# sfu-rsl/FastTrack

Measured on AMD Instinct MI355X. Metric: frames/sec extract+match, higher is better.
Workload: dtype u8

## Files before the change

fasttrack_amd/csrc/kernels_extract.hip:

```cpp
#include "ft_internal.h"
#include "libm_f32.h"
#include "wave_ops.h"

namespace {


struct FtMomentTab {
    unsigned W[17 * 8], M[17 * 8];
};
constexpr FtMomentTab ft_make_moment_tab() {
    constexpr int umax[16] = {15, 15, 15, 15, 14, 14, 14, 13, 13, 12, 11, 10, 9, 8, 6, 3};
    FtMomentTab t{};
    for (int av = 0; av < 16; av++)
        for (int j = 0; j < 8; j++)
            for (int k = 0; k < 4; k++) {
                const int u = -15 + 4 * j + k;
                const int au = u < 0 ? -u : u;
                if (u <= 15 && au <= umax[av]) {
                    t.W[av * 8 + j] |= (unsigned)(u + 16) << (8 * k);
                    t.M[av * 8 + j] |= 1u << (8 * k);
                }
            }
    return t;
}
// ... 140 lines not shown
                pk |= (unsigned)((r0[0] + r0[1] + r1[0] + r1[1] + 2) >> 2) << (8 * k);
            }
            gstore<unsigned>(outLevel + (unsigned)vmad24(dy, D.pitch, bx), pk);
        }
        return;
    }
    int cx0[4], cx1[4];
#pragma unroll
    for (int k = 0; k < 4; k++) {
        cx0[k] = xt[k].s - sxa;
        cx1[k] = min(xt[k].s + 1, sw - 1) - sxa;
    }
#pragma unroll
    for (int j = 0; j < 4; j++) {
        const int dy = by + j;
        if (dy > dy1) break;
        const int sy0 = min(max((int)yt[j].s, 0), sh - 1) - sya, sy1 = min(max((int)yt[j].s + 1, 0), sh - 1) - sya;
        const uint8_t *r0 = T + __mul24(sy0, ldsPitch), *r1 = T + __mul24(sy1, ldsPitch);
        unsigned pk = 0;
#pragma unroll
        for (int k = 0; k < 4; k++) {
            const int h0 = r0[cx0[k]] * xt[k].a0 + r0[cx1[k]] * xt[k].a1;
            const int h1 = r1[cx0[k]] * xt[k].a0 + r1[cx1[k]] * xt[k].a1;
            pk |= (unsigned)(((vmul24((int)yt[j].a0, h0 >> 4) >> 16) + (vmul24((int)yt[j].a1, h1 >> 4) >> 16) + 2) >> 2) << (8 * k);
        }
        gstore<unsigned>(outLevel + (unsigned)vmad24(dy, D.pitch, bx), pk);
    }
}

#define PR_COLS 128
#ifndef PR_RB
#define PR_RB 32
#endif
#ifndef PR_PF
#define PR_PF 4
#endif
typedef unsigned short ft_us2 __attribute__((ext_vector_type(2)));
typedef unsigned ft_u2 __attribute__((ext_vector_type(2)));
__device__ __forceinline__ unsigned udot2_u16(unsigned a, unsigned b) {
    return __builtin_amdgcn_udot2(__builtin_bit_cast(ft_us2, a), __builtin_bit_cast(ft_us2, b), 0u, false);
}
__device__ __forceinline__ unsigned umulhi_su(unsigned bShifted16, unsigned a) {
    unsigned r;
    asm("v_mul_hi_u32 %0, %1, %2" : "=v"(r) : "s"(bShifted16), "v"(a));
    return r;
}
template <bool AREA, bool BAND>
__device__ __forceinline__ void pyr_rows_strip(const FtGeom &g, int level, int slot, int tx, int j0, int rowEnd, int lane,
                                               const uint8_t *S, int spitch, uint8_t *pyr, const FtTap *taps, int readableEnd) {
    const FtLevelGeom &D = g.lv[level];
    const int sw = g.lv[level - 1].w, sh = g.lv[level - 1].h;
    const int dx = tx * PR_COLS + 2 * lane;
    const int nrows = min(PR_RB, (BAND ? rowEnd : D.h) - j0);
    unsigned rowW0 = 0, rowW1 = 0;
    if constexpr (!AREA) {
        const ft_u2 t = gload<ft_u2>(taps + D.ytab + j0 + min(lane, nrows - 1));
        const int sy = (int)(short)(t.x & 0xffffu);
        rowW0 = (unsigned)min(max(sy, 0), sh - 1) | ((unsigned)min(max(sy + 1, 0), sh - 1) << 16);
        rowW1 = (t.x >> 16) | (t.y << 16);
        if (lane >= nrows) rowW0 = 0xffffffffu;
    }
    const int dxa = min(dx, D.w - 1), dxb = min(dx + 1, D.w - 1);
    int sxa, sxb, cxa, cxb;
    unsigned wa, wb;
    if constexpr (AREA) {
        sxa = 2 * dxa; sxb = 2 * dxb; cxa = sxa + 1; cxb = sxb + 1;
        wa = wb = 0x00010001u;
    } else {
        const ft_u2 ta = gload<ft_u2>(taps + D.xtab + dxa), tb = gload<ft_u2>(taps + D.xtab + dxb);
        sxa = (int)(short)(ta.x & 0xffffu); sxb = (int)(short)(tb.x & 0xffffu);
        cxa = min(sxa + 1, sw - 1); cxb = min(sxb + 1, sw - 1);
        wa = (ta.x >> 16) | (ta.y << 16);
        wb = (tb.x >> 16) | (tb.y << 16);
    }
    const int base = min(sxa & ~3, readableEnd - 8);
    const unsigned selA = (unsigned)(sxa - base) | 0x0c00u | ((unsigned)(cxa - base) << 16) | 0x0c000000u;
    const unsigned selB = (unsigned)(sxb - base) | 0x0c00u | ((unsigned)(cxb - base) << 16) | 0x0c000000u;
    auto rowTap = [&](int r, int &sy0, int &sy1, unsigned &b0, unsigned &b1) {
        if constexpr (AREA) {
            sy0 = 2 * (j0 + r); sy1 = r < nrows ? sy0 + 1 : -1; b0 = b1 = 0;
        } else {
            const unsigned w0 = (unsigned)__builtin_amdgcn_readlane((int)rowW0, r), w1 = (unsigned)__builtin_amdgcn_readlane((int)rowW1, r);
            sy0 = (int)(w0 & 0xffffu); sy1 = (int)(w0 >> 16);
            b0 = w1 << 16; b1 = w1 & 0xffff0000u;
        }
    };
    int jr = 0, sy0, sy1;
    unsigned b0, b1;
    rowTap(0, sy0, sy1, b0, b1);
    int lastSy0, rLast;
    unsigned bx0, bx1;
    rowTap(nrows - 1, lastSy0, rLast, bx0, bx1);
    int r = sy0;
    const uint8_t *srcBase = S;
    uint8_t *dstBase = pyr + (size_t)slot * g.pyrPerSlot + D.off + (size_t)j0 * D.pitch;
    unsigned dOff = 0;
    const unsigned laneSrc = (unsigned)base, laneDst = (unsigned)dx;
    const bool store2 = dx + 1 < D.w, store1 = dx < D.w;
    auto run = [&](auto edgeTag) {
        constexpr bool EDGE = decltype(edgeTag)::value;
        int pfIdx = r;
        auto prefetch = [&]() -> ft_u2 {
            unsigned offS = laneSrc + (unsigned)min(pfIdx, rLast) * (unsigned)spitch;
            asm volatile("" : "+v"(offS));
            const ft_u2 v = gload<ft_u2>(srcBase + offS);
            pfIdx++;
            return v;
        };
        ft_u2 q[PR_PF];
#pragma unroll
        for (int k = 0; k < PR_PF; k++) q[k] = prefetch();
        unsigned hpA = 0, hpB = 0, hcA = 0, hcB = 0;
        auto take = [&](ft_u2 &q) {
            hpA = hcA; hpB = hcB;
            hcA = udot2_u16(__builtin_amdgcn_perm(q.y, q.x, selA), wa);
            hcB = udot2_u16(__builtin_amdgcn_perm(q.y, q.x, selB), wb);
            if constexpr (!AREA) { hcA >>= 4; hcB >>= 4; }
            q = prefetch();
        };
        auto step = [&]() {
            while (sy1 == r) {
                if (__builtin_expect(sy0 == r, 0)) {
                    hpA = hcA; hpB = hcB;
                    asm volatile("" : "+v"(hpA), "+v"(hpB));
                }
                unsigned oA, oB;
                if constexpr (AREA) {
                    oA = (hpA + hcA + 2u) >> 2; oB = (hpB + hcB + 2u) >> 2;
                } else {
                    oA = (umulhi_su(b0, hpA) + umulhi_su(b1, hcA) + 2u) >> 2;
                    oB = (umulhi_su(b0, hpB) + umulhi_su(b1, hcB) + 2u) >> 2;
                }
                unsigned offD = laneDst + dOff;
                asm volatile("" : "+v"(offD));
                if constexpr (!EDGE) {
                    gstore<unsigned short>(dstBase + offD, (unsigned short)(oA | (oB << 8)));
                } else {
                    if (store2) gstore<unsigned short>(dstBase + offD, (unsigned short)(oA | (oB << 8)));
                    else if (store1) gstore<uint8_t>(dstBase + offD, (uint8_t)oA);
                }
                dOff += (unsigned)D.pitch;
                jr++;
                rowTap(jr, sy0, sy1, b0, b1);
            }
            r++;
        };
        for (int left = rLast - r + 1; left > 0; left -= PR_PF) {
#pragma unroll
            for (int k = 0; k < PR_PF; k++) {
                take(q[k]);
                step();
            }
        }
    };
    if (tx * PR_COLS + PR_COLS <= D.w) run(std::false_type{});
    else run(std::true_type{});
}

template <bool AREA>
__global__ __launch_bounds__(64) void k_pyr_rows(FtGeom g, int level, const uint8_t *const *l0, int l0pitch, uint8_t *pyr,
                                                 const FtTap *taps, FtSlotGrid sg, int stripsX, unsigned sxMagic,
                                                 int readableEnd) {
    const int lane = threadIdx.x;
    int slot, tile;
    if (!ft_slot_block(sg, slot, tile)) return;
    const int ty = div_by(tile, sxMagic), tx = tile - ty * stripsX;
    int spitch;
    const uint8_t *S = level_ptr(g, level - 1, slot, l0, l0pitch, pyr, spitch);
    pyr_rows_strip<AREA, false>(g, level, slot, tx, ty * PR_RB, 0, lane, S, spitch, pyr, taps, readableEnd);
}

__global__ __launch_bounds__(64 * PC_WAVES) void k_pyr_cascade(FtGeom g, const uint8_t *const *l0, int l0pitch, uint8_t *pyr,
                                                              const FtTap *taps, FtSlotGrid sg, FtPyrBands pb,
                                                              int l0ReadableEnd) {
    const int lane = threadIdx.x & 63, wave = wave_index();
    int slot, band;
    if (!ft_slot_block(sg, slot, band)) return;
    const uint8_t *const frame = l0[slot];
    for (int level = 1; level < g.nlevels; level++) {
        const unsigned rr = pb.rows[level][band];
        const int r0 = (int)(rr & 0xffffu), r1 = (int)(rr >> 16);
        const int stripsX = (g.lv[level].w + PR_COLS - 1) / PR_COLS;
        const unsigned sxMagic = div_magic_small((unsigned)stripsX);
        const int n = stripsX * ((r1 - r0 + PR_RB - 1) / PR_RB);
        const int readableEnd = level == 1 ? l0ReadableEnd : g.lv[level - 1].pitch;
        const int spitch = level == 1 ? l0pitch : g.lv[level - 1].pitch;
        const uint8_t *S = level == 1 ? frame : pyr + (size_t)slot * g.pyrPerSlot + g.lv[level - 1].off;
        for (int s = wave; s < n; s += PC_WAVES) {
            const int ty = div_by(s, sxMagic), tx = s - ty * stripsX;
            const int j0 = r0 + ty * PR_RB;
            if (g.lv[level].area2x) pyr_rows_strip<true, true>(g, level, slot, tx, j0, r1, lane, S, spitch, pyr, taps, readableEnd);
            else pyr_rows_strip<false, true>(g, level, slot, tx, j0, r1, lane, S, spitch, pyr, taps, readableEnd);
        }
        if (level + 1 < g.nlevels) {
            __builtin_amdgcn_fence(__ATOMIC_RELEASE, "workgroup");
            __syncthreads();
            __builtin_amdgcn_fence(__ATOMIC_ACQUIRE, "workgroup");
        }
    }
}

typedef unsigned short fs_us2 __attribute__((ext_vector_type(2)));
__device__ __forceinline__ unsigned pk_max_u16(unsigned a, unsigned b) {
    return __builtin_bit_cast(unsigned, __builtin_elementwise_max(__builtin_bit_cast(fs_us2, a), __builtin_bit_cast(fs_us2, b)));
}
__device__ __forceinline__ unsigned pk_min_u16(unsigned a, unsigned b) {
    return __builtin_bit_cast(unsigned, __builtin_elementwise_min(__builtin_bit_cast(fs_us2, a), __builtin_bit_cast(fs_us2, b)));
}
__device__ __forceinline__ bool has_arc9(unsigned m) {
    unsigned d = m | (m << 16);
    unsigned a = d & (d >> 1);
    a &= a >> 2;
    a &= a >> 4;
    a &= d >> 8;
    return (a & 0xffffu) != 0;
}

#define FT_RING(F)                                                                                            \
    F(0, 0, 3) F(1, 1, 3) F(2, 2, 2) F(3, 3, 1) F(4, 3, 0) F(5, 3, -1) F(6, 2, -2) F(7, 1, -3) F(8, 0, -3)    \
    F(9, -1, -3) F(10, -2, -2) F(11, -3, -1) F(12, -3, 0) F(13, -3, 1) F(14, -2, 2) F(15, -1, 3)

__device__ __forceinline__ int fast_score(int v, const int p[16]) {
    int mn3[16], mx3[16];
#pragma unroll
    for (int k = 0; k < 16; k++) {
        mn3[k] = min(min(p[k], p[(k + 1) & 15]), p[(k + 2) & 15]);
        mx3[k] = max(max(p[k], p[(k + 1) & 15]), p[(k + 2) & 15]);
    }
    int mn9[16], mx9[16];
#pragma unroll
    for (int k = 0; k < 16; k++) {
        mn9[k] = min(min(mn3[k], mn3[(k + 3) & 15]), mn3[(k + 6) & 15]);
        mx9[k] = max(max(mx3[k], mx3[(k + 3) & 15]), mx3[(k + 6) & 15]);
    }
    int darkest = max(max(mn9[0], mn9[1]), mn9[2]), brightest = min(min(mx9[0], mx9[1]), mx9[2]);
#pragma unroll
    for (int k = 3; k < 15; k += 2) {
        darkest = max(max(darkest, mn9[k]), mn9[k + 1]);
        brightest = min(min(brightest, mx9[k]), mx9[k + 1]);
    }
    darkest = max(darkest, mn9[15]);
    brightest = min(brightest, mx9[15]);
    return max(v - brightest, darkest - v) - 1;
}

__device__ __forceinline__ unsigned pk_min3_h(unsigned a, unsigned b, unsigned c) {
    unsigned r;
    asm("v_pk_minimum3_f16 %0, %1, %2, %3" : "=v"(r) : "v"(a), "v"(b), "v"(c));
    return r;
}
__device__ __forceinline__ unsigned pk_max3_h(unsigned a, unsigned b, unsigned c) {
    unsigned r;
    asm("v_pk_maximum3_f16 %0, %1, %2, %3" : "=v"(r) : "v"(a), "v"(b), "v"(c));
    return r;
}
typedef short fs_s2 __attribute__((ext_vector_type(2)));
__device__ __forceinline__ unsigned fast_score2(unsigned v, const unsigned p[16]) {
    unsigned mn3[16], mx3[16];
#pragma unroll
    for (int k = 0; k < 16; k++) {
        mn3[k] = pk_min3_h(p[k], p[(k + 1) & 15], p[(k + 2) & 15]);
        mx3[k] = pk_max3_h(p[k], p[(k + 1) & 15], p[(k + 2) & 15]);
    }
    unsigned mn9[16], mx9[16];
#pragma unroll
    for (int k = 0; k < 16; k++) {
        mn9[k] = pk_min3_h(mn3[k], mn3[(k + 3) & 15], mn3[(k + 6) & 15]);
        mx9[k] = pk_max3_h(mx3[k], mx3[(k + 3) & 15], mx3[(k + 6) & 15]);
    }
    unsigned darkest = pk_max3_h(mn9[0], mn9[1], mn9[2]), brightest = pk_min3_h(mx9[0], mx9[1], mx9[2]);
#pragma unroll
    for (int k = 3; k < 15; k += 2) {
        darkest = pk_max3_h(darkest, mn9[k], mn9[k + 1]);
        brightest = pk_min3_h(brightest, mx9[k], mx9[k + 1]);
    }
    const fs_s2 dk = __builtin_bit_cast(fs_s2, pk_max3_h(darkest, mn9[15], mn9[15]));
    const fs_s2 br = __builtin_bit_cast(fs_s2, pk_min3_h(brightest, mx9[15], mx9[15]));
    const fs_s2 vv = __builtin_bit_cast(fs_s2, v);
    const fs_s2 sc = __builtin_elementwise_max(vv - br, dk - vv) - (fs_s2)(1);
    return __builtin_bit_cast(unsigned, sc);
}

#ifndef FC_CAND
#define FC_CAND 512
#endif
#ifndef FC_XCD_RUN
#define FC_XCD_RUN 8
#endif
#ifndef FC_UNROLL
#define FC_UNROLL 2
#endif
#ifndef FC_ROWS
#define FC_ROWS 4
#endif
#ifndef FC_NMS_REG
#define FC_NMS_REG 2
#endif
#ifndef FC_CORN
#define FC_CORN 384
#endif
#ifndef FC_WAVES_PER_EU
#define FC_WAVES_PER_EU 1
#endif
__host__ __device__ __forceinline__ int fc_pitch(int wCell, int TP) { return TP ? TP : ((wCell + 12) & ~3); }
__host__ __device__ __forceinline__ int fc_tile_bytes(int wCell, int hCell, int TP) {
    const int t = (hCell + 6) * fc_pitch(wCell, TP), f = wCell * hCell;
    return ((t > f ? t : f) + 15) & ~15;
}
__host__ __device__ __forceinline__ int fc_score_bytes(int wCell, int hCell, int TP) { return (((hCell + 2) * fc_pitch(wCell, TP)) + 15) & ~15; }
__host__ __device__ __forceinline__ int fc_list_bytes() { return 2 * (FC_CAND + FC_CORN) + 16; }

template <int TP, bool ORDERED>
__global__ __launch_bounds__(64, FC_WAVES_PER_EU) void k_fast_cells(FtGeom g, const uint8_t *const *l0, int l0pitch, const uint8_t *pyr,
                                                   int iniTh, int minTh, int alignedLoads, int *cellCount,
                                                   uint32_t *stage, const FtCellRec *cellTab, FtSlotGrid sg, int dbg, int tileBytes,
                                                   int scoreBytesMax, FtCellRanges cr) {
    extern __shared__ __attribute__((aligned(16))) uint8_t smem[];
    const int lane = threadIdx.x;
    int slot = blockIdx.y, cellSg = 0;
    if (sg.xcdMap && !ft_slot_block(sg, slot, cellSg)) return;
    const uint8_t *img0 = l0[slot];
    const int j = (int)(blockIdx.x >> 3), xcd = (int)(blockIdx.x & 7);
    const int cj = sg.xcdMap ? cellSg : ((j / FC_XCD_RUN) * 8 + xcd) * FC_XCD_RUN + (j % FC_XCD_RUN);
    if (cj >= cr.n0 + cr.n1) return;
    const int cell = cj < cr.n0 ? cr.lo0 + cj : cr.lo1 + (cj - cr.n0);
    const FtCellRec rec = cellTab[cell];
    const int iniX = (int)(rec.origin & 0xffffu), iniY = (int)(rec.origin >> 16);
    const int tw = (int)(rec.shape & 0xffu), th = (int)((rec.shape >> 8) & 0xffu), level = (int)((rec.shape >> 16) & 0xffu);
    int *cnt = cellCount + (size_t)slot * g.totalCells + cell;
    if (tw == 0) {
        if (lane == 0) *cnt = 0;
        return;
    }
    const unsigned lv = g.fastLv[level];
    const int cellCap = (int)(lv >> 16);
    const int pw = tw - 6, ph = th - 6;
    const int npx = pw * ph;
    const int tp = TP ? TP : fc_pitch(g.lv[level].wCell, 0);
    const unsigned pwMagic = TP ? 0u : div_magic_of((unsigned)pw);
    uint8_t *tile = smem;
    uint8_t *score = tile + (TP ? tileBytes : fc_tile_bytes(g.lv[level].wCell, g.lv[level].hCell, 0));
    const int scoreBytes = TP ? ((ph + 2) * TP + 15) & ~15 : fc_score_bytes(g.lv[level].wCell, g.lv[level].hCell, 0);
    unsigned short *cand = (unsigned short *)(score + (TP ? scoreBytesMax : scoreBytes));
    unsigned short *corn = cand + FC_CAND;
    const int pitch = level ? (int)(lv & 0xffffu) : l0pitch;
    const uint8_t *org = level ? pyr + ((size_t)slot * g.pyrPerSlot + rec.srcOff) : img0 + ((size_t)iniY * l0pitch + iniX);
    int ax = 0;
    if (alignedLoads) {
        ax = iniX & 3;
        const int nd = (tw + ax + 3) >> 2;
        const uint8_t *src = org - ax;
        if constexpr (TP != 0) {
            constexpr int DW = TP / 4, RPT = 64 / DW;
            const int rr = lane / DW, cc4 = 4 * min(lane - rr * DW, nd - 1);
            if (th > 8 * RPT && th <= 9 * RPT) {
                const unsigned goff = (unsigned)vmad24(rr, pitch, cc4);
                unsigned *tl = (unsigned *)(tile + vmad24(rr, TP, cc4));
                const int row8 = min(8 * RPT + rr, th - 1);
                unsigned v[9];
#pragma unroll
                for (int k = 0; k < 8; k++) v[k] = gload<unsigned>(src + (goff + (unsigned)(k * RPT * pitch)));
                v[8] = gload<unsigned>(src + (unsigned)vmad24(row8, pitch, cc4));
#pragma unroll
                for (int k = 0; k < 8; k++) tl[k * RPT * (TP / 4)] = v[k];
                *(unsigned *)(tile + vmad24(row8, TP, cc4)) = v[8];
            } else
            for (int r0 = 0; r0 < th; r0 += 9 * RPT) {
                unsigned v[9];
                int row[9];
#pragma unroll
                for (int k = 0; k < 9; k++) {
                    row[k] = min(r0 + k * RPT + rr, th - 1);
                    v[k] = gload<unsigned>(src + (unsigned)vmad24(row[k], pitch, cc4));
                }
#pragma unroll
                for (int k = 0; k < 9; k++) *(unsigned *)(tile + vmad24(row[k], TP, cc4)) = v[k];
            }
        } else {
            const unsigned ndMagic = div_magic_of((unsigned)nd);
            for (int i0 = 0; i0 < nd * th; i0 += 64 * 9) {
                unsigned v[9];
                int off[9];
#pragma unroll
                for (int k = 0; k < 9; k++) {
                    const int i = i0 + 64 * k + lane, ic = min(i, nd * th - 1);
                    const int y = div_by(ic, ndMagic), x = ic - y * nd;
                    off[k] = i < nd * th ? y * tp + 4 * x : -1;
                    v[k] = gload<unsigned>(src + (size_t)y * pitch + 4 * x);
                }
#pragma unroll
                for (int k = 0; k < 9; k++)
                    if (off[k] >= 0) *(unsigned *)(tile + off[k]) = v[k];
            }
        }
    } else {
        const unsigned twMagic = div_magic_of((unsigned)tw);
        const uint8_t *src = org;
        for (int i = lane; i < tw * th; i += 64) {
            const int y = div_by(i, twMagic), x = i - y * tw;
            tile[y * tp + x] = gload<uint8_t>(src + (size_t)y * pitch + x);
        }
    }
    for (int i = lane; i < scoreBytes >> 4; i += 64) ((uint4 *)score)[i] = make_uint4(0, 0, 0, 0);
    wave_lds_sync();
    if (dbg & 4) {
        if (lane == 0) *cnt = (int)tile[lane] & 0;
        return;
    }
    const uint8_t *t0 = tile + ax;
    int nc = 0, ncorn = 0;
    auto pixCode = [&](int y, int x) -> int { return TP > 0 ? ((y << 6) | x) : y * pw + x; };
    auto pixY = [&](int code) -> int { return TP > 0 ? code >> 6 : div_by(code, pwMagic); };
    auto pixX = [&](int code, int y) -> int { return TP > 0 ? (code & 63) : code - y * pw; };
    auto flushB = [&]() {
        if (dbg & 16) {
            nc = 0;
            return;
        }
        wave_lds_sync();
        int jb = 0;
        if constexpr (TP > 0) {
            for (; nc - jb > 64 && !(dbg & 9); jb += 128) {
                const int jA = jb + lane, jB = jb + 64 + lane;
                const int cA = cand[jA], cB = cand[min(jB, nc - 1)];
                const int yA = pixY(cA), xA = pixX(cA, yA), yB = pixY(cB), xB = pixX(cB, yB);
                const uint8_t *wA = t0 + yA * tp + xA, *wB = t0 + yB * tp + xB;
                unsigned v2;
                unsigned ring2[16];
                v2 = (unsigned)wA[3 * tp + 3] | ((unsigned)wB[3 * tp + 3] << 16);
#define FT_LD2(k, ox, oy) ring2[k] = (unsigned)wA[((oy) + 3) * tp + (ox) + 3] | ((unsigned)wB[((oy) + 3) * tp + (ox) + 3] << 16);
                FT_RING(FT_LD2)
#undef FT_LD2
                const unsigned sc2 = fast_score2(v2, ring2);
                const int scA = (int)(short)(sc2 & 0xffffu), scB = (int)(short)(sc2 >> 16);
                const bool cornA = scA >= minTh, cornB = scB >= minTh;
                score[(yA + 1) * tp + (xA + 1)] = (uint8_t)(cornA ? scA : 0);
                score[(yB + 1) * tp + (xB + 1)] = (uint8_t)(cornB ? scB : 0);
                const bool isB = cornB && jB < nc;
                const unsigned long long ba = __builtin_amdgcn_ballot_w64(cornA), bb = __builtin_amdgcn_ballot_w64(isB);
                const int posA = (int)__builtin_amdgcn_mbcnt_hi((unsigned)(ba >> 32), __builtin_amdgcn_mbcnt_lo((unsigned)ba, (unsigned)ncorn));
                ncorn += __popcll(ba);
                const int posB = (int)__builtin_amdgcn_mbcnt_hi((unsigned)(bb >> 32), __builtin_amdgcn_mbcnt_lo((unsigned)bb, (unsigned)ncorn));
                ncorn += __popcll(bb);
                corn[cornA && posA < FC_CORN ? posA : FC_CORN] = (unsigned short)cA;
                corn[isB && posB < FC_CORN ? posB : FC_CORN] = (unsigned short)cB;
            }
        }
        for (; jb < nc; jb += 64) {
            const int j = jb + lane;
            const int ci2 = cand[min(j, nc - 1)];
            const int y = pixY(ci2), x = pixX(ci2, y);
            const uint8_t *win = t0 + y * tp + x;
            const int v = win[3 * tp + 3];
            int ringPx[16];
#define FT_LD(k, ox, oy) ringPx[k] = (int)win[((oy) + 3) * tp + (ox) + 3];
            FT_RING(FT_LD)
#undef FT_LD
            const int sc = (dbg & 1) ? ((v + ringPx[0] + ringPx[5] + ringPx[11]) & 31) : fast_score(v, ringPx);
            const bool corner = sc >= minTh;
            score[(y + 1) * tp + (x + 1)] = (uint8_t)(corner ? sc : 0);
            const bool isCorner = corner && j < nc;
            const unsigned long long cb = __builtin_amdgcn_ballot_w64(isCorner);
            const int pos = (int)__builtin_amdgcn_mbcnt_hi((unsigned)(cb >> 32), __builtin_amdgcn_mbcnt_lo((unsigned)cb, (unsigned)ncorn));
            corn[isCorner && pos < FC_CORN ? pos : FC_CORN] = (unsigned short)ci2;
            ncorn += __popcll(cb);
        }
        nc = 0;
        wave_lds_sync();
    };
#define FT_AD(ox, oy) __builtin_amdgcn_sad_u8(v, (unsigned)cpx[(oy)*tp + (ox)], 0u)
    auto pushRow = [&](bool pass, int code, int n) -> int {
        const unsigned long long b = __ballot(pass);
        const int pos = pass ? (int)__builtin_amdgcn_mbcnt_hi((unsigned)(b >> 32), __builtin_amdgcn_mbcnt_lo((unsigned)b, (unsigned)n))
                             : FC_CAND + FC_CORN;
        cand[pos] = (unsigned short)code;
        return n + __popcll(b);
    };
    if constexpr (TP > 0 && !ORDERED) {
        const int half = lane >> 5, cx = lane & 31;
        const int hRows = (ph + 1) >> 1;
        const int y0h = half * hRows;
        const int wMain = min(pw, 32);
        const bool actC = cx < wMain;
        const uint8_t *col = t0 + min(cx, wMain - 1) + 3 + y0h * TP;
        const int codeBase = (y0h << 6) | cx;
        unsigned pA = col[3 * TP], pB = col[4 * TP], pC = col[5 * TP];
        unsigned hist0 = __builtin_amdgcn_sad_hi_u8(pA, (unsigned)col[0], 0u);
        unsigned hist1 = __builtin_amdgcn_sad_hi_u8(pC, (unsigned)col[2 * TP], __builtin_amdgcn_sad_u8(pB, (unsigned)col[TP], 0u));
        const unsigned th = (unsigned)minTh;
        const int rowsHalf = half ? ph - hRows : hRows;
        for (int yb = 0; yb < hRows; yb += 28) {
        const int yEnd = min(yb + 28, hRows);
        unsigned cmask = 0;
        auto trip = [&](int y) {
            const uint8_t *r = col + y * TP;
            unsigned pv[7];
            pv[0] = pA; pv[1] = pB; pv[2] = pC;
#pragma unroll
            for (int k = 0; k < 4; k++) pv[k + 3] = r[(k + 6) * TP];
            const unsigned ps0 = __builtin_amdgcn_sad_hi_u8(pv[1], pv[4], __builtin_amdgcn_sad_u8(pv[0], pv[3], 0u));
            const unsigned ps1 = __builtin_amdgcn_sad_hi_u8(pv[3], pv[6], __builtin_amdgcn_sad_u8(pv[2], pv[5], 0u));
            const unsigned pn0 = __builtin_amdgcn_alignbit(hist1, hist0, 16);
            const unsigned pn1 = __builtin_amdgcn_alignbit(ps0, hist1, 16);
            const unsigned pe0 = __builtin_amdgcn_sad_hi_u8(pv[1], (unsigned)r[4 * TP + 3], __builtin_amdgcn_sad_u8(pv[0], (unsigned)r[3 * TP + 3], 0u));
            const unsigned pw0 = __builtin_amdgcn_sad_hi_u8(pv[1], (unsigned)r[4 * TP - 3], __builtin_amdgcn_sad_u8(pv[0], (unsigned)r[3 * TP - 3], 0u));
            const unsigned pe1 = __builtin_amdgcn_sad_hi_u8(pv[3], (unsigned)r[6 * TP + 3], __builtin_amdgcn_sad_u8(pv[2], (unsigned)r[5 * TP + 3], 0u));
            const unsigned pw1 = __builtin_amdgcn_sad_hi_u8(pv[3], (unsigned)r[6 * TP - 3], __builtin_amdgcn_sad_u8(pv[2], (unsigned)r[5 * TP - 3], 0u));
            const unsigned M0 = pk_min_u16(pk_max_u16(pn0, ps0), pk_max_u16(pe0, pw0));
            const unsigned M1 = pk_min_u16(pk_max_u16(pn1, ps1), pk_max_u16(pe1, pw1));
            hist0 = ps0; hist1 = ps1;
            pA = pv[4]; pB = pv[5]; pC = pv[6];
            asm("v_cmp_gt_u32_sdwa vcc, %1, %2 src0_sel:WORD_0 src1_sel:DWORD\n\tv_addc_co_u32 %0, vcc, %0, %0, vcc\n\t"
                "v_cmp_gt_u32_sdwa vcc, %1, %2 src0_sel:WORD_1 src1_sel:DWORD\n\tv_addc_co_u32 %0, vcc, %0, %0, vcc\n\t"
                "v_cmp_gt_u32_sdwa vcc, %3, %2 src0_sel:WORD_0 src1_sel:DWORD\n\tv_addc_co_u32 %0, vcc, %0, %0, vcc\n\t"
                "v_cmp_gt_u32_sdwa vcc, %3, %2 src0_sel:WORD_1 src1_sel:DWORD\n\tv_addc_co_u32 %0, vcc, %0, %0, vcc"
                : "+v"(cmask)
                : "v"(M0), "v"(th), "v"(M1)
                : "vcc");
        };
        int y = yb;
        for (; y + 4 < yEnd; y += 8) {
            trip(y);
            trip(y + 4);
        }
        if (y < yEnd) trip(y);
        {
            const int T = (yEnd - yb + 3) & ~3;
            const int cnt = min(max(rowsHalf - yb, 0), T);
            const unsigned valid = actC ? (((1u << cnt) - 1u) << (T - cnt)) : 0u;
            cmask &= valid;
            const int codeTop = codeBase + ((yb + T - 1) << 6);
            int incl = __popc(cmask);
            const int own = incl;
            incl += __builtin_amdgcn_update_dpp(0, incl, 0x111, 0xF, 0xF, true);
            incl += __builtin_amdgcn_update_dpp(0, incl, 0x112, 0xF, 0xF, true);
            incl += __builtin_amdgcn_update_dpp(0, incl, 0x114, 0xF, 0xF, true);
            incl += __builtin_amdgcn_update_dpp(0, incl, 0x118, 0xF, 0xF, true);
            incl += __builtin_amdgcn_update_dpp(0, incl, 0x142, 0xA, 0xF, true);
            incl += __builtin_amdgcn_update_dpp(0, incl, 0x143, 0xC, 0xF, true);
            const int total = __builtin_amdgcn_readlane(incl, 63);
            if (nc + total > FC_CAND - 64) flushB();
            if (total <= FC_CAND - 64) {
                unsigned short *slot = cand + (nc + incl - own);
                while (__builtin_amdgcn_ballot_w64(cmask != 0u)) {
                    *(cmask ? slot : cand + (FC_CAND + FC_CORN)) = (unsigned short)(codeTop - (__builtin_ctz(cmask | 0x80000000u) << 6));
                    cmask &= cmask - 1u;
                    slot++;
                }
                nc += total;
            } else {
                for (;;) {
                    const unsigned long long b = __builtin_amdgcn_ballot_w64(cmask != 0u);
                    if (!b) break;
                    const int pos = (int)__builtin_amdgcn_mbcnt_hi((unsigned)(b >> 32), __builtin_amdgcn_mbcnt_lo((unsigned)b, (unsigned)nc));
                    const int bit = __builtin_ctz(cmask | 0x80000000u);
                    if (__builtin_amdgcn_inverse_ballot_w64(b)) cand[pos] = (unsigned short)(codeTop - (bit << 6));
                    cmask &= cmask - 1u;
                    nc += __popcll(b);
                    if (nc > FC_CAND - 64) flushB();
                }
            }
        }
        }
        const int wRem = pw - wMain, nRem = wRem * ph;
        if (wRem > 0) {
            const unsigned remMagic = div_magic_small((unsigned)wRem);
            for (int base = 0; base < nRem; base += 64) {
                const int i = base + lane;
                const int ii = min(i, nRem - 1);
                const int yy = div_by(ii, remMagic), xx = wMain + ii - yy * wRem;
                const uint8_t *cpx = t0 + (yy + 3) * TP + (xx + 3);
                const unsigned v = cpx[0];
                const unsigned m0 = max(FT_AD(0, 3), FT_AD(0, -3));
                const unsigned m1 = max(FT_AD(3, 0), FT_AD(-3, 0));
                const unsigned m01r = i < nRem ? min(m0, m1) : 0u;
                if (__any(m01r > (unsigned)minTh)) nc = pushRow(m01r > (unsigned)minTh, pixCode(yy, xx), nc);
                if (nc > FC_CAND - 64) flushB();
            }
        }
        flushB();
    } else if constexpr (TP > 0) {
        const bool act = lane < pw;
        const uint8_t *col = t0 + min(lane, pw - 1) + 3;
        unsigned pA = col[3 * TP], pB = col[4 * TP], pC = col[5 * TP];
        unsigned dA = __builtin_amdgcn_sad_u8(pA, (unsigned)col[0], 0u);
        unsigned dB = __builtin_amdgcn_sad_u8(pB, (unsigned)col[TP], 0u);
        unsigned dC = __builtin_amdgcn_sad_u8(pC, (unsigned)col[2 * TP], 0u);
        for (int y = 0; y < ph; y += FC_ROWS) {
            const uint8_t *r = col + y * TP;
            unsigned pv[FC_ROWS + 3], m01[FC_ROWS], dSv[FC_ROWS], mAny = 0;
            pv[0] = pA; pv[1] = pB; pv[2] = pC;
#pragma unroll
            for (int k = 0; k < FC_ROWS; k++) pv[k + 3] = r[(k + 6) * TP];
#pragma unroll
            for (int k = 0; k < FC_ROWS; k++) {
                const unsigned v = pv[k];
                const uint8_t *cpx = r + (k + 3) * TP;
                const unsigned dS = dSv[k] = __builtin_amdgcn_sad_u8(v, pv[k + 3], 0u);
                const unsigned dN = k == 0 ? dA : k == 1 ? dB : k == 2 ? dC : dSv[k >= 3 ? k - 3 : 0];
                const unsigned m1 = max(FT_AD(3, 0), FT_AD(-3, 0));
                m01[k] = (act && y + k < ph) ? min(max(dN, dS), m1) : 0u;
                mAny = max(mAny, m01[k]);
            }
            dA = dSv[FC_ROWS - 3]; dB = dSv[FC_ROWS - 2]; dC = dSv[FC_ROWS - 1];
            pA = pv[FC_ROWS]; pB = pv[FC_ROWS + 1]; pC = pv[FC_ROWS + 2];
            if (__any(mAny > (unsigned)minTh)) {
#pragma unroll
                for (int k = 0; k < FC_ROWS; k++) nc = pushRow(m01[k] > (unsigned)minTh, pixCode(y + k, lane), nc);
            }
            if (nc > FC_CAND - FC_ROWS * 64 || y + FC_ROWS >= ph) flushB();
        }
    } else {
        for (int base = 0; base < npx; base += 64 * FC_UNROLL) {
            unsigned m01[FC_UNROLL];
            const uint8_t *cp[FC_UNROLL];
            unsigned mAny = 0;
#pragma unroll
            for (int u = 0; u < FC_UNROLL; u++) {
                const int i = base + 64 * u + lane;
                const int ii = min(i, npx - 1);
                const int y = div_by(ii, pwMagic), x = ii - y * pw;
                const uint8_t *cpx = t0 + (y + 3) * tp + (x + 3);
                cp[u] = cpx;
                const unsigned v = cpx[0];
                const unsigned m0 = max(FT_AD(0, 3), FT_AD(0, -3));
                const unsigned m1 = max(FT_AD(3, 0), FT_AD(-3, 0));
                m01[u] = i < npx ? min(m0, m1) : 0u;
                mAny = max(mAny, m01[u]);
            }
            if (__any(mAny > (unsigned)minTh)) {
#pragma unroll
                for (int u = 0; u < FC_UNROLL; u++) {
                    const int i = base + 64 * u + lane;
                    const uint8_t *cpx = cp[u];
                    const unsigned v = cpx[0];
                    const unsigned m2 = max(FT_AD(2, 2), FT_AD(-2, -2));
                    const unsigned m3 = max(FT_AD(2, -2), FT_AD(-2, 2));
                    const bool pass = min(m01[u], min(m2, m3)) > (unsigned)minTh;
                    const unsigned long long b = __ballot(pass);
                    if (pass) cand[nc + __popcll(b & ((1ull << lane) - 1ull))] = (unsigned short)i;
                    nc += __popcll(b);
                }
            }
            if (nc > FC_CAND - 64 * FC_UNROLL || base + 64 * FC_UNROLL >= npx) flushB();
        }
    }
#undef FT_AD
    wave_lds_sync();
    if (dbg & 2) {
        if (lane == 0) *cnt = 0;
        return;
    }
    const bool useList = ncorn <= FC_CORN;
    const int nItems = useList ? ncorn : npx;
    auto nms = [&](int item, int &pix) -> int {
        int y, x;
        if (useList) {
            pix = (int)corn[item];
            y = pixY(pix), x = pixX(pix, y);
        } else {
            const unsigned mg = TP ? div_magic_of((unsigned)pw) : pwMagic;
            y = div_by(item, mg), x = item - y * pw;
            pix = pixCode(y, x);
        }
        const uint8_t *s = score + y * tp + x;
        const unsigned v = s[tp + 1];
        const unsigned m = max(max(max(max((unsigned)s[0], (unsigned)s[1]), (unsigned)s[2]),
                                   max(max((unsigned)s[tp], (unsigned)s[tp + 2]), (unsigned)s[2 * tp])),
                               max((unsigned)s[2 * tp + 1], (unsigned)s[2 * tp + 2]));
        return v > m ? (v >= (unsigned)iniTh ? 2 : 1) : 0;
    };
    uint32_t *out = stage + ((size_t)slot * g.stagePerSlot + rec.outOff);
    int run = 0;
    auto emit = [&](int fl, int pix, int need) {
        const bool f = fl >= need;
        const unsigned long long b = __builtin_amdgcn_ballot_w64(f);
        const int y = pixY(pix), x = pixX(pix, y);
        const int pos = (int)__builtin_amdgcn_mbcnt_hi((unsigned)(b >> 32), __builtin_amdgcn_mbcnt_lo((unsigned)b, (unsigned)run));
        const uint32_t packed = ft_pack_cand(x + (iniX - 13), y + (iniY - 13), score[(y + 1) * tp + (x + 1)]);
        if (f && pos < cellCap) out[pos] = packed;
        run += __popcll(b);
    };
    if (nItems <= 64 * FC_NMS_REG) {
        int fl[FC_NMS_REG], px[FC_NMS_REG], anyHi = 0;
#pragma unroll
        for (int q = 0; q < FC_NMS_REG; q++) {
            fl[q] = 0;
            px[q] = 0;
            if (q * 64 < nItems) {
                const int f = nms(min(q * 64 + lane, nItems - 1), px[q]);
                fl[q] = q * 64 + lane < nItems ? f : 0;
                anyHi |= __any(fl[q] == 2);
            }
        }
        const int need = anyHi ? 2 : 1;
#pragma unroll
        for (int q = 0; q < FC_NMS_REG; q++)
            if (q * 64 < nItems) emit(fl[q], px[q], need);
    } else {
        auto itemPix = [&](int it) -> int {
            if (useList) return (int)corn[it];
            const unsigned mg = TP ? div_magic_of((unsigned)pw) : pwMagic;
            const int y = div_by(it, mg);
            return pixCode(y, it - y * pw);
        };
        unsigned mx = 0;
        for (int base = 0; base < nItems; base += 64) {
            const int pix = itemPix(min(base + lane, nItems - 1));
            const int y = pixY(pix), x = pixX(pix, y);
            mx = max(mx, (unsigned)score[(y + 1) * tp + (x + 1)]);
        }
        int need = __any(mx >= (unsigned)iniTh) ? 2 : 1;
        for (;;) {
            int anyHi = 0;
            run = 0;
            for (int base = 0; base < nItems; base += 64) {
                const int it = base + lane;
                int pix = 0;
                const int f = nms(min(it, nItems - 1), pix);
                const int fl = it < nItems ? f : 0;
                anyHi |= __any(fl == 2);
                emit(fl, pix, need);
            }
            if (need == 1 || anyHi) break;
            need = 1;
        }
    }
    if (lane == 0) *cnt = min(run, cellCap);
}

__global__ __launch_bounds__(256) void k_compact(FtGeom g, const int *cellCount, const uint32_t *stage,
                                                 uint32_t *cand, int *candCount) {
    extern __shared__ __attribute__((aligned(16))) uint8_t smem[];
    int *offs = (int *)smem;
    __shared__ int wsum[4];
    const int tid = threadIdx.x, lane = tid & 63, wave = tid >> 6;
    const int level = blockIdx.x, slot = blockIdx.y;
    const FtLevelGeom &L = g.lv[level];
    const int nCells = L.nCols * L.nRows;
    const int *cnt = cellCount + (size_t)slot * g.totalCells + L.cellBase;
    const int per = (nCells + 255) / 256;
    const int c0 = tid * per, c1 = min(c0 + per, nCells);
    int local = 0;
    for (int c = c0; c < c1; c++) local += cnt[c];
    int incl = local;
#pragma unroll
    for (int o = 1; o < 64; o <<= 1) {
        int t = __shfl_up(incl, o);
        if (lane >= o) incl += t;
    }
    if (lane == 63) wsum[wave] = incl;
    __syncthreads();
    int wbase = 0, total = 0;
#pragma unroll
    for (int w = 0; w < 4; w++) {
        if (w < wave) wbase += wsum[w];
        total += wsum[w];
    }
    int run = wbase + incl - local;
    for (int c = c0; c < c1; c++) {
        offs[c] = run;
        run += cnt[c];
    }
    if (tid == 0) offs[nCells] = total;
    __syncthreads();
    total = min(total, L.candCap);
    const uint32_t *st = stage + (size_t)slot * g.stagePerSlot + L.stageBase;
    uint32_t *dst = cand + (size_t)slot * g.candPerSlot + L.candBase;
    for (int o = tid; o < total; o += 256) {
        int lo = 0, hi = nCells;
        while (hi - lo > 1) {
            int mid = (lo + hi) >> 1;
            if (offs[mid] <= o) lo = mid;
            else hi = mid;
        }
        dst[o] = st[(size_t)lo * L.cellCap + (o - offs[lo])];
    }
    if (tid == 0) candCount[slot * g.nlevels + level] = total;
}

#define OD_R 21
#define OD_P (2 * OD_R + 1)
#define OD_PP 48
#define OD_HP 40
#ifndef OD_LAYOUT
#define OD_LAYOUT 1
#endif
#ifndef OD_RP
#define OD_RP 44
#endif
#define OD_RAW_BYTES (OD_P * OD_PP)
#define OD_HB_BYTES (OD_LAYOUT ? OD_HP * OD_RP * 2 + 16 : OD_P * OD_HP * 2)
#define OD_WAVE_BYTES ((OD_RAW_BYTES + OD_HB_BYTES + 15) & ~15)
#define OD_WAVES 4
#ifndef OD_MFMA
#define OD_MFMA 0
#endif
#if OD_MFMA && !OD_LAYOUT
#error "OD_MFMA writes the column-major layout"
#endif
#define OD_BIAS (OD_MFMA ? 0x80808080u : 0u)
#ifndef OD_KPW_WIDE
#define OD_KPW_WIDE 2
#endif

__device__ __forceinline__ int reflect101(int i, int n) {
    if (i < 0) i = -i;
    if (i >= n) i = 2 * (n - 1) - i;
    return i;
}

__device__ __forceinline__ void od_hblur4(unsigned d0, unsigned d1, unsigned d2, unsigned &h0, unsigned &h1, unsigned &h2, unsigned &h3) {
#define FT_W4(a, b, c, d) ((unsigned)(a) | ((unsigned)(b) << 8) | ((unsigned)(c) << 16) | ((unsigned)(d) << 24))
    const unsigned W0a = FT_W4(18, 34, 48, 56), W0b = FT_W4(48, 34, 18, 0);
    const unsigned W1a = FT_W4(0, 18, 34, 48), W1b = FT_W4(56, 48, 34, 18);
    const unsigned W2a = FT_W4(0, 0, 18, 34), W2b = FT_W4(48, 56, 48, 34), W2c = FT_W4(18, 0, 0, 0);
    const unsigned W3a = FT_W4(0, 0, 0, 18), W3b = FT_W4(34, 48, 56, 48), W3c = FT_W4(34, 18, 0, 0);
#undef FT_W4
    h0 = __builtin_amdgcn_udot4(d1, W0b, __builtin_amdgcn_udot4(d0, W0a, 0u, false), false);
    h1 = __builtin_amdgcn_udot4(d1, W1b, __builtin_amdgcn_udot4(d0, W1a, 0u, false), false);
    h2 = __builtin_amdgcn_udot4(d2, W2c, __builtin_amdgcn_udot4(d1, W2b, __builtin_amdgcn_udot4(d0, W2a, 0u, false), false), false);
    h3 = __builtin_amdgcn_udot4(d2, W3c, __builtin_amdgcn_udot4(d1, W3b, __builtin_amdgcn_udot4(d0, W3a, 0u, false), false), false);
}
__device__ __forceinline__ unsigned od_vblur7(unsigned p0, unsigned p1, unsigned p2, unsigned p3, unsigned p4, unsigned p5, unsigned p6) {
    unsigned v;
    asm("v_mad_u32_u24 %0, %1, 18, %2" : "=v"(v) : "v"(p0 + p6), "s"(32768u));
    asm("v_mad_u32_u24 %0, %1, 34, %2" : "=v"(v) : "v"(p1 + p5), "v"(v));
    asm("v_mad_u32_u24 %0, %1, 48, %2" : "=v"(v) : "v"(p2 + p4), "v"(v));
    asm("v_mad_u32_u24 %0, %1, 56, %2" : "=v"(v) : "v"(p3), "v"(v));
    return v >> 16;
}

typedef unsigned short od_us2 __attribute__((ext_vector_type(2)));
typedef int od_v4i __attribute__((ext_vector_type(4)));
__device__ __forceinline__ unsigned od_dot2(unsigned a, unsigned w, unsigned acc) {
    return __builtin_amdgcn_udot2(__builtin_bit_cast(od_us2, a), __builtin_bit_cast(od_us2, w), acc, false);
}
__device__ __forceinline__ unsigned od_vblur7_pairs(unsigned e0, unsigned e1, unsigned e2, unsigned e3) {
    const unsigned W01 = 18u | (34u << 16), W23 = 48u | (56u << 16), W45 = 48u | (34u << 16), W6 = 18u;
    return od_dot2(e3, W6, od_dot2(e2, W45, od_dot2(e1, W23, od_dot2(e0, W01, 32768u)))) >> 16;
}
__device__ __forceinline__ unsigned od_vblur7_dwords(unsigned d0, unsigned d1, unsigned d2, unsigned d3, unsigned sh) {
    return od_vblur7_pairs(__builtin_amdgcn_alignbit(d1, d0, sh), __builtin_amdgcn_alignbit(d2, d1, sh),
                           __builtin_amdgcn_alignbit(d3, d2, sh), d3 >> (sh & 31u));
}

typedef short od_s2 __attribute__((ext_vector_type(2)));
__device__ __forceinline__ int od_sdot2(unsigned a, unsigned w, int acc) {
    return __builtin_amdgcn_sdot2(__builtin_bit_cast(od_s2, a), __builtin_bit_cast(od_s2, w), acc, false);
}
__device__ __forceinline__ unsigned od_vblur7_dwords_s(unsigned d0, unsigned d1, unsigned d2, unsigned d3, unsigned sh) {
    const unsigned W01 = 18u | (34u << 16), W23 = 48u | (56u << 16), W45 = 48u | (34u << 16), W6 = 18u;
    const unsigned e0 = __builtin_amdgcn_alignbit(d1, d0, sh), e1 = __builtin_amdgcn_alignbit(d2, d1, sh),
                   e2 = __builtin_amdgcn_alignbit(d3, d2, sh), e3 = d3 >> (sh & 31u);
    return (unsigned)od_sdot2(e3, W6, od_sdot2(e2, W45, od_sdot2(e1, W23, od_sdot2(e0, W01, 32768 + 256 * 32768)))) >> 16;
}

__global__ void k_blur_level(const uint8_t *img, int pitch, int w, int h, uint8_t *dst, int dstPitch) {
    const int gx = (blockIdx.x * blockDim.x + threadIdx.x) * 4, y = blockIdx.y;
    if (gx >= w || y >= h) return;
    unsigned hb[7][4];
    for (int s = 0; s < 7; s++) {
        const uint8_t *row = img + (size_t)reflect101(y + s - 3, h) * pitch;
        unsigned d[3] = {0u, 0u, 0u};
        for (int b = 0; b < 12; b++) d[b >> 2] |= (unsigned)row[reflect101(gx - 3 + b, w)] << (8 * (b & 3));
        od_hblur4(d[0], d[1], d[2], hb[s][0], hb[s][1], hb[s][2], hb[s][3]);
    }
    for (int j = 0; j < 4 && gx + j < w; j++) {
#if OD_LAYOUT
        const unsigned t[8] = {hb[0][j], hb[1][j], hb[2][j], hb[3][j], hb[4][j], hb[5][j], hb[6][j], 0u};
        unsigned v;
        if ((gx + j + y) & 1) v = od_vblur7_dwords(t[0] << 16, t[1] | (t[2] << 16), t[3] | (t[4] << 16), t[5] | (t[6] << 16), 16u);
        else v = od_vblur7_dwords(t[0] | (t[1] << 16), t[2] | (t[3] << 16), t[4] | (t[5] << 16), t[6], 0u);
        dst[(size_t)y * dstPitch + gx + j] = (uint8_t)v;
#else
        dst[(size_t)y * dstPitch + gx + j] = (uint8_t)od_vblur7(hb[0][j], hb[1][j], hb[2][j], hb[3][j], hb[4][j], hb[5][j], hb[6][j]);
#endif
    }
}

__device__ __forceinline__ float fast_atan2_deg(float y, float x) {
// ... 549 lines not shown
```

Before: 82910.

## Fold remainder-column FAST test into banded main loop and lean per-lane append

Removes the separate per-pixel pass over columns beyond 32. Those columns are now handled inside the main row-band loop: lanes are assigned vertical bands of the remainder columns and run the same SAD-based 4-row trip, and their masks are merged into the same prefix-sum append. The append skips entirely when no lane has candidates, uses a per-lane divergent store loop instead of a wave-wide ballot loop, and builds the valid-row mask with med3/bfm. This cuts loop overhead and extra barriers, but adds divergence and more complex index math, and candidate order may change.

```diff
diff --git a/fasttrack_amd/csrc/kernels_extract.hip b/fasttrack_amd/csrc/kernels_extract.hip
--- a/fasttrack_amd/csrc/kernels_extract.hip
+++ b/fasttrack_amd/csrc/kernels_extract.hip
@@ -466,6 +466,9 @@
 #ifndef FC_WAVES_PER_EU
 #define FC_WAVES_PER_EU 1
 #endif
+#ifndef FC_LEAN_APPEND
+#define FC_LEAN_APPEND 1
+#endif
 __host__ __device__ __forceinline__ int fc_pitch(int wCell, int TP) { return TP ? TP : ((wCell + 12) & ~3); }
 __host__ __device__ __forceinline__ int fc_tile_bytes(int wCell, int hCell, int TP) {
     const int t = (hCell + 6) * fc_pitch(wCell, TP), f = wCell * hCell;
@@ -652,12 +655,22 @@
         unsigned hist0 = __builtin_amdgcn_sad_hi_u8(pA, (unsigned)col[0], 0u);
         unsigned hist1 = __builtin_amdgcn_sad_hi_u8(pC, (unsigned)col[2 * TP], __builtin_amdgcn_sad_u8(pB, (unsigned)col[TP], 0u));
         const unsigned th = (unsigned)minTh;
-        const int rowsHalf = half ? ph - hRows : hRows;
-        for (int yb = 0; yb < hRows; yb += 28) {
-        const int yEnd = min(yb + 28, hRows);
-        unsigned cmask = 0;
-        auto trip = [&](int y) {
-            const uint8_t *r = col + y * TP;
+        const int rowsHalf = actC ? (half ? ph - hRows : hRows) : 0;
+        auto validMask = [](int cnt, int n, int T) -> unsigned {
+            int c;
+            unsigned m;
+            asm("v_med3_i32 %0, %1, 0, %2" : "=v"(c) : "v"(cnt), "s"(n));
+            asm("v_bfm_b32 %0, %1, %2" : "=v"(m) : "v"(c), "v"(T - c));
+            return m;
+        };
+        const int wRem = pw - wMain;
+        const unsigned remMagic = div_magic_small((unsigned)wRem);
+        int nbR = 0, bR = 0;
+        if (wRem > 0) {
+            nbR = div_by(64, remMagic);
+            bR = div_by(ph + nbR - 1, div_magic_small((unsigned)nbR));
+        }
+        auto trip4 = [&](const uint8_t *r, unsigned &pA, unsigned &pB, unsigned &pC, unsigned &hist0, unsigned &hist1, unsigned &cmask) {
             unsigned pv[7];
             pv[0] = pA; pv[1] = pB; pv[2] = pC;
 #pragma unroll
@@ -682,19 +695,39 @@
                 : "v"(M0), "v"(th), "v"(M1)
                 : "vcc");
         };
+        for (int yb = 0; yb < hRows; yb += 28) {
+        const int yEnd = min(yb + 28, hRows);
+        unsigned cmask = 0;
+        auto trip = [&](int y) { trip4(col + y * TP, pA, pB, pC, hist0, hist1, cmask); };
         int y = yb;
         for (; y + 4 < yEnd; y += 8) {
             trip(y);
             trip(y + 4);
         }
         if (y < yEnd) trip(y);
-        {
-            const int T = (yEnd - yb + 3) & ~3;
-            const int cnt = min(max(rowsHalf - yb, 0), T);
-            const unsigned valid = actC ? (((1u << cnt) - 1u) << (T - cnt)) : 0u;
-            cmask &= valid;
-            const int codeTop = codeBase + ((yb + T - 1) << 6);
-            int incl = __popc(cmask);
+        unsigned rmask = 0;
+        int codeTopR = 0;
+        if (yb < bR) {
+            int laneR = lane;
+            asm volatile("" : "+v"(laneR));
+            const int band = div_by(laneR, remMagic), rc = vmad24(band, -wRem, laneR);
+            const int yy = vmad24(band, bR, yb);
+            const uint8_t *rcol = (t0 + 35) + vmad24(min(yy, ph), TP, rc);
+            unsigned qA = rcol[3 * TP], qB = rcol[4 * TP], qC = rcol[5 * TP];
+            unsigned h0 = __builtin_amdgcn_sad_hi_u8(qA, (unsigned)rcol[0], 0u);
+            unsigned h1 = __builtin_amdgcn_sad_hi_u8(qC, (unsigned)rcol[2 * TP], __builtin_amdgcn_sad_u8(qB, (unsigned)rcol[TP], 0u));
+            const int nR = min(bR - yb, 28);
+            trip4(rcol, qA, qB, qC, h0, h1, rmask);
+            for (int yr = 4; yr < nR; yr += 4) trip4(rcol + (unsigned)(yr * TP), qA, qB, qC, h0, h1, rmask);
+            const int TR = (nR + 3) & ~3;
+            rmask &= validMask(ph - yy, nR, TR);
+            codeTopR = ((yy << 6) + rc) + (((TR - 1) << 6) + 32);
+        }
+        const int T = (yEnd - yb + 3) & ~3;
+        cmask &= validMask(rowsHalf - yb, T, T);
+        const int codeTop = codeBase + ((yb + T - 1) << 6);
+        if (!FC_LEAN_APPEND || __builtin_amdgcn_ballot_w64((cmask | rmask) != 0u)) {
+            int incl = __popc(cmask) + __popc(rmask);
             const int own = incl;
             incl += __builtin_amdgcn_update_dpp(0, incl, 0x111, 0xF, 0xF, true);
             incl += __builtin_amdgcn_update_dpp(0, incl, 0x112, 0xF, 0xF, true);
@@ -706,41 +739,47 @@
             if (nc + total > FC_CAND - 64) flushB();
             if (total <= FC_CAND - 64) {
                 unsigned short *slot = cand + (nc + incl - own);
-                while (__builtin_amdgcn_ballot_w64(cmask != 0u)) {
-                    *(cmask ? slot : cand + (FC_CAND + FC_CORN)) = (unsigned short)(codeTop - (__builtin_ctz(cmask | 0x80000000u) << 6));
-                    cmask &= cmask - 1u;
-                    slot++;
-                }
+#if FC_LEAN_APPEND
+                auto append = [&](unsigned m, int top) {
+                    if (m) {
+                        do {
+                            *slot = (unsigned short)vmad24(__builtin_ctz(m), -64, top);
+                            slot++;
+                            m &= m - 1u;
+                        } while (m);
+                    }
+                };
+#else
+                auto append = [&](unsigned m, int top) {
+                    unsigned short *s = slot;
+                    slot += __popc(m);
+                    while (__builtin_amdgcn_ballot_w64(m != 0u)) {
+                        *(m ? s : cand + (FC_CAND + FC_CORN)) = (unsigned short)(top - (__builtin_ctz(m | 0x80000000u) << 6));
+                        m &= m - 1u;
+                        s++;
+                    }
+                };
+#endif
+                append(cmask, codeTop);
+                append(rmask, codeTopR);
                 nc += total;
             } else {
-                for (;;) {
-                    const unsigned long long b = __builtin_amdgcn_ballot_w64(cmask != 0u);
-                    if (!b) break;
-                    const int pos = (int)__builtin_amdgcn_mbcnt_hi((unsigned)(b >> 32), __builtin_amdgcn_mbcnt_lo((unsigned)b, (unsigned)nc));
-                    const int bit = __builtin_ctz(cmask | 0x80000000u);
-                    if (__builtin_amdgcn_inverse_ballot_w64(b)) cand[pos] = (unsigned short)(codeTop - (bit << 6));
-                    cmask &= cmask - 1u;
-                    nc += __popcll(b);
-                    if (nc > FC_CAND - 64) flushB();
+                for (int part = 0; part < 2; part++) {
+                    unsigned m = part ? rmask : cmask;
+                    const int top = part ? codeTopR : codeTop;
+                    for (;;) {
+                        const unsigned long long b = __builtin_amdgcn_ballot_w64(m != 0u);
+                        if (!b) break;
+                        const int pos = (int)__builtin_amdgcn_mbcnt_hi((unsigned)(b >> 32), __builtin_amdgcn_mbcnt_lo((unsigned)b, (unsigned)nc));
+                        const int bit = __builtin_ctz(m | 0x80000000u);
+                        if (__builtin_amdgcn_inverse_ballot_w64(b)) cand[pos] = (unsigned short)(top - (bit << 6));
+                        m &= m - 1u;
+                        nc += __popcll(b);
+                        if (nc > FC_CAND - 64) flushB();
+                    }
                 }
             }
         }
-        }
-        const int wRem = pw - wMain, nRem = wRem * ph;
-        if (wRem > 0) {
-            const unsigned remMagic = div_magic_small((unsigned)wRem);
-            for (int base = 0; base < nRem; base += 64) {
-                const int i = base + lane;
-                const int ii = min(i, nRem - 1);
-                const int yy = div_by(ii, remMagic), xx = wMain + ii - yy * wRem;
-                const uint8_t *cpx = t0 + (yy + 3) * TP + (xx + 3);
-                const unsigned v = cpx[0];
-                const unsigned m0 = max(FT_AD(0, 3), FT_AD(0, -3));
-                const unsigned m1 = max(FT_AD(3, 0), FT_AD(-3, 0));
-                const unsigned m01r = i < nRem ? min(m0, m1) : 0u;
-                if (__any(m01r > (unsigned)minTh)) nc = pushRow(m01r > (unsigned)minTh, pixCode(yy, xx), nc);
-                if (nc > FC_CAND - 64) flushB();
-            }
         }
         flushB();
     } else if constexpr (TP > 0) {
```

Measured after the change: 84220 (median of 6 runs). +1.6%, better.
